# cemlyn007/ale-libtorch-ppo

Hardware: AMD Instinct MI355X
Metric: env steps/sec (whole node), Breakout 84x84x4 (higher is better)
Workload: dtype bf16; 1 GPU; Breakout-shaped synthetic, 128 envs/GPU x T=128, A=4, H=512, 4 epochs x 4 minibatches of 4096 (configs[1], v0.yaml update shape); envs_per_gpu=128, horizon=128, epochs=4, minibatches=4, parallelism=dp1, frames=raw u8 [E,2,210,160] pairs resident in HBM, rollout_planes=fp32, update_graph=False, dp_schedule_forced=False

## Files before the change

### ale-libtorch-ppo_amd/csrc/gemm_launch.hip

```cpp
#include "common.hpp"
#include "gemm.hpp"
#include "gemm_pipe.hpp"
#include <algorithm>
#include <cstdlib>

namespace aleppo {

static int tune(const char *name, int dflt) {
  const char *e = std::getenv(name);
  return e ? std::atoi(e) : dflt;
}
static inline dim3 grid2(long M, int BM, long N, int BN, int Z = 1) {
  return dim3((unsigned)((M + BM - 1) / BM), (unsigned)((N + BN - 1) / BN), (unsigned)Z);
}

template <class T, bool IDX = false>
static void conv1_fwd_t(hipStream_t s, const uint32_t *obs, SampleMap map, const void *W1, const float *b1, void *a1,
                        long ns) {
  if constexpr (!IDX)
    if (map.idx)
      return conv1_fwd_t<T, true>(s, obs, map, W1, b1, a1, ns);
  using AL = ConvGatherLoader<T, uint8_t, 400, 20, 4, 84, 4, 8, IDX>;
  using BL = DenseLoader<T>;
  using EP = EpiBiasAct<T, true>;
  const long M = ns * 400;
  typename AL::P ap{reinterpret_cast<const uint8_t *>(obs), map.TP, map.s1 * 4, map.s0 * 4, map.base * 4, map.n0, map.idx};
  typename BL::P bp{static_cast<const T *>(W1), 256, 0};
  typename EP::P ep{static_cast<T *>(a1), b1, 32, 1.0f / 255.0f};
  hipLaunchKernelGGL((gemm_nt_kernel<T, AL, BL, EP, 128, 32, 4, 1>), grid2(M, 128, 32, 32), dim3(256), 0, s, ap, bp,
                     ep, (int)M, 32, 256);
}
template <class T>
static void conv2_fwd_t(hipStream_t s, const void *a1, const void *W2, const float *b2, void *a2, long ns) {
  using AL = ConvGatherLoader<T, T, 81, 9, 2, 20, 32, 4>;
  using BL = DenseLoader<T>;
  using EP = EpiBiasAct<T, true>;
  const long M = ns * 81;
  typename AL::P ap{static_cast<const T *>(a1), 1, 400 * 32, 0, 0, 0};
  typename BL::P bp{static_cast<const T *>(W2), 512, 0};
  typename EP::P ep{static_cast<T *>(a2), b2, 64, 1.0f};
  hipLaunchKernelGGL((gemm_nt_kernel<T, AL, BL, EP, 128, 64, 2, 2>), grid2(M, 128, 64, 64), dim3(256), 0, s, ap, bp,
                     ep, (int)M, 64, 512);
}
template <class T>
static void conv3_fwd_t(hipStream_t s, const void *a2, const void *W3, const float *b3, void *a3, long ns) {
  using AL = ConvGatherLoader<T, T, 49, 7, 1, 9, 64, 3>;
  using BL = DenseLoader<T>;
  using EP = EpiBiasAct<T, true>;
  const long M = ns * 49;
  typename AL::P ap{static_cast<const T *>(a2), 1, 81 * 64, 0, 0, 0};
  typename BL::P bp{static_cast<const T *>(W3), 576, 0};
  typename EP::P ep{static_cast<T *>(a3), b3, 64, 1.0f};
  hipLaunchKernelGGL((gemm_nt_kernel<T, AL, BL, EP, 128, 64, 2, 2>), grid2(M, 128, 64, 64), dim3(256), 0, s, ap, bp,
                     ep, (int)M, 64, 576);
}

static int pipe_cus() {
  static int n = 0;
  if (!n) {
    int dev = 0;
    hipDeviceProp_t p;
    if (hipGetDevice(&dev) == hipSuccess && hipGetDeviceProperties(&p, dev) == hipSuccess)
      n = p.multiProcessorCount;
    if (n <= 0)
      n = 256;
  }
  return n;
}
template <int MODE, int NST> static void launch_pipe(hipStream_t s, const PipeParams &P) {
  static bool once = false;
  constexpr size_t sm = gemm_pipe_smem<MODE, NST>();
  static_assert(sm <= 160 * 1024, "LDS budget");
  if (!once) {
    (void)hipFuncSetAttribute(reinterpret_cast<const void *>(gemm_pipe_kernel<MODE, NST>),
                              hipFuncAttributeMaxDynamicSharedMemorySize, (int)sm);
    once = true;
  }
  const int cus = pipe_cus() / 8 * 8, rounds = (P.njobs + cus - 1) / cus;
  const int grid = P.njobs >= cus / 4 ? std::min(cus, ((P.njobs + rounds - 1) / rounds + 7) / 8 * 8) : std::min(P.njobs, cus);
  hipLaunchKernelGGL((gemm_pipe_kernel<MODE, NST>), dim3(grid), dim3(PIPE_THREADS), sm, s, P);
}
static bool fc_dma() {
  static const bool v = tune("ALEPPO_FC_DMA", 1) != 0;
  return v;
}
static bool tn_xcd() {
  static const bool v = tune("ALEPPO_TN_XCD", 1) != 0;
  return v;
}
static bool use_pipe() { return tuning().fc_pipe; }
static int fc_fwd_pipe(hipStream_t s, const void *a3, const void *Wfc, const float *bfc, float *h, long ns, int H,
                       int max_parts) {
  const int tm = (int)((ns + 127) / 128), tn = (H + 127) / 128, tiles = tm * tn, cus = pipe_cus();
  int best = 1;
  double best_t = 1e30;
  for (int sp = 1; sp <= max_parts; ++sp) {
    const double t = (double)((tiles * sp + cus - 1) / cus) / sp + 0.02 * sp;
    if (t < best_t - 1e-9) {
      best_t = t;
      best = sp;
    }
  }
  PipeParams P{};
  P.A = static_cast<const bf16 *>(a3);
  P.lda = FC_IN;
  P.B = static_cast<const bf16 *>(Wfc);
  P.ldb = FC_IN;
  P.M = (int)ns;
  P.N = H;
  P.tiles_m = tm;
  P.tiles_n = tn;
  P.nstages = FC_IN / 64;
  P.splits = best;
  P.njobs = tiles * best;
  P.out_f32 = h;
  P.bias = bfc;
  launch_pipe<0, 4>(s, P);
  return best;
}
static void fc_dgrad_pipe(hipStream_t s, const void *dh, const void *WfcT, const void *a3, void *dz3, long ns, int H) {
  PipeParams P{};
  P.A = static_cast<const bf16 *>(dh);
  P.lda = H;
  P.B = static_cast<const bf16 *>(WfcT);
  P.ldb = H;
  P.M = (int)ns;
  P.N = FC_IN;
  P.tiles_m = (int)((ns + 127) / 128);
  P.tiles_n = (FC_IN + 127) / 128;
  P.nstages = H / 64;
  P.splits = 1;
  P.njobs = P.tiles_m * P.tiles_n;
  P.out_bf16 = static_cast<bf16 *>(dz3);
  P.gate = static_cast<const bf16 *>(a3);
  launch_pipe<1, 4>(s, P);
}
template <class T>
static void fc_fwd_t(hipStream_t s, const void *a3, const void *Wfc, const float *bfc, float *h, long ns, int H) {
  using AL = DenseLoader<T>;
  using BL = DenseLoader<T>;
  using EP = EpiBiasAct<float, false>;
  typename AL::P ap{static_cast<const T *>(a3), FC_IN, 0};
  typename BL::P bp{static_cast<const T *>(Wfc), FC_IN, 0};
  typename EP::P ep{h, bfc, H, 1.0f};
  if (ns <= 256)
    hipLaunchKernelGGL((gemm_nt_kernel<T, AL, BL, EP, 32, 32, 2, 2>), grid2(ns, 32, H, 32), dim3(256), 0, s, ap, bp,
                       ep, (int)ns, H, FC_IN);
  else if (fc_dma() && FC_IN % Atom<T>::KT == 0) {
    static const int v = tune("ALEPPO_FC_FWD_TILE", 1);
    const T *a = static_cast<const T *>(a3), *b = static_cast<const T *>(Wfc);
    if (v == 3 && FC_IN % (2 * Atom<T>::KT) == 0)
      hipLaunchKernelGGL((gemm_nt_dma_kernel<T, EP, 64, 64, 2, 2, 16>), grid2(ns, 64, H, 64), dim3(256), 0, s, a, FC_IN,
                         b, FC_IN, ep, (int)ns, H, FC_IN);
    else if (v == 4 && FC_IN % (2 * Atom<T>::KT) == 0)
      hipLaunchKernelGGL((gemm_nt_dma_kernel<T, EP, 128, 64, 2, 2, 16>), grid2(ns, 128, H, 64), dim3(256), 0, s, a,
                         FC_IN, b, FC_IN, ep, (int)ns, H, FC_IN);
    else if (v == 1)
      hipLaunchKernelGGL((gemm_nt_dma_kernel<T, EP, 64, 64, 2, 2>), grid2(ns, 64, H, 64), dim3(256), 0, s, a, FC_IN, b,
                         FC_IN, ep, (int)ns, H, FC_IN);
    else if (v == 2)
      hipLaunchKernelGGL((gemm_nt_dma_kernel<T, EP, 128, 128, 2, 2>), grid2(ns, 128, H, 128), dim3(256), 0, s, a,
                         FC_IN, b, FC_IN, ep, (int)ns, H, FC_IN);
    else
      hipLaunchKernelGGL((gemm_nt_dma_kernel<T, EP, 128, 64, 2, 2>), grid2(ns, 128, H, 64), dim3(256), 0, s, a, FC_IN,
                         b, FC_IN, ep, (int)ns, H, FC_IN);
  } else {
    static const int v = tune("ALEPPO_FC_FWD_TILE", 1);
    if (v == 1)
      hipLaunchKernelGGL((gemm_nt_kernel<T, AL, BL, EP, 64, 64, 2, 2>), grid2(ns, 64, H, 64), dim3(256), 0, s, ap, bp,
                         ep, (int)ns, H, FC_IN);
    else if (v == 2)
      hipLaunchKernelGGL((gemm_nt_kernel<T, AL, BL, EP, 128, 128, 2, 2>), grid2(ns, 128, H, 128), dim3(256), 0, s, ap,
                         bp, ep, (int)ns, H, FC_IN);
    else if (v == 3)
      hipLaunchKernelGGL((gemm_nt_kernel<T, AL, BL, EP, 64, 128, 2, 2>), grid2(ns, 64, H, 128), dim3(256), 0, s, ap,
                         bp, ep, (int)ns, H, FC_IN);
    else
      hipLaunchKernelGGL((gemm_nt_kernel<T, AL, BL, EP, 128, 64, 2, 2>), grid2(ns, 128, H, 64), dim3(256), 0, s, ap,
                         bp, ep, (int)ns, H, FC_IN);
  }
}

template <class T> static void fc_fwd_splitk_t(hipStream_t s, const void *a3, const void *Wfc, float *hpart, long ns, int H) {
  using AL = DenseLoader<T>;
  using BL = DenseLoader<T>;
  using EP = EpiPartial;
  constexpr int KC = FC_IN / FC_SPLITS;
  typename AL::P ap{static_cast<const T *>(a3), FC_IN, KC};
  typename BL::P bp{static_cast<const T *>(Wfc), FC_IN, KC};
  typename EP::P ep{hpart, H, ns * (long)H};
  hipLaunchKernelGGL((gemm_nt_kernel<T, AL, BL, EP, 32, 32, 2, 2>), grid2(ns, 32, H, 32, FC_SPLITS), dim3(256), 0, s,
                     ap, bp, ep, (int)ns, H, KC);
}
__global__ __launch_bounds__(256) void fc_act_kernel(const bf16 *__restrict__ a3, const bf16 *__restrict__ Wfc,
                                                     float *__restrict__ hpart, int M, int N) {
  constexpr int KC = FC_IN / FC_SPLITS, KS = KC / 32, VPR = KC / 8;
  constexpr int ROWV = VPR + 1;
  constexpr int NV = 32 * VPR / 256;
  __shared__ u32x4 sA[32 * ROWV], sB[32 * ROWV];
  const int tid = threadIdx.x, lane = tid & 63, wave = tid >> 6, fr = lane & 15, fg = lane >> 4;
  const int wm = wave >> 1, wn = wave & 1, z = blockIdx.z;
  const int m0 = blockIdx.x * 32, n0 = blockIdx.y * 32;
  u32x4 ra[NV], rb[NV];
#pragma unroll
  for (int i = 0; i < NV; ++i) {
    const int v = tid + 256 * i, r = v / VPR, c = v - r * VPR;
    ra[i] = *reinterpret_cast<const u32x4 *>(a3 + (long)min(m0 + r, M - 1) * FC_IN + z * KC + c * 8);
    rb[i] = *reinterpret_cast<const u32x4 *>(Wfc + (long)min(n0 + r, N - 1) * FC_IN + z * KC + c * 8);
  }
#pragma unroll
  for (int i = 0; i < NV; ++i) {
    const int v = tid + 256 * i, r = v / VPR, c = v - r * VPR;
    sA[r * ROWV + c] = ra[i];
    sB[r * ROWV + c] = rb[i];
  }
  __syncthreads();
  f32x4 acc = {0.f, 0.f, 0.f, 0.f};
#pragma unroll
  for (int ks = 0; ks < KS; ++ks)
    Atom<bf16>::mma(sA[(wm * 16 + fr) * ROWV + ks * 4 + fg], sB[(wn * 16 + fr) * ROWV + ks * 4 + fg], acc);
  float *out = hpart + (long)z * M * N;
  const int nn = n0 + wn * 16 + fr;
#pragma unroll
  for (int r = 0; r < 4; ++r) {
    const int mm = m0 + wm * 16 + fg * 4 + r;
    if (mm < M && nn < N)
      out[(long)mm * N + nn] = acc[r];
  }
}
void fc_fwd_splitk(hipStream_t s, int prec, const void *a3, const void *Wfc, float *hpart, long ns, int H) {
  static const bool latency_form = tune("ALEPPO_FC_ACT_LATENCY", 1) != 0;
  if (prec == ALEPPO_BF16 && latency_form)
    hipLaunchKernelGGL(fc_act_kernel, grid2(ns, 32, H, 32, FC_SPLITS), dim3(256), 0, s, static_cast<const bf16 *>(a3),
                       static_cast<const bf16 *>(Wfc), hpart, (int)ns, H);
  else if (prec == ALEPPO_BF16)
    fc_fwd_splitk_t<bf16>(s, a3, Wfc, hpart, ns, H);
  else
    fc_fwd_splitk_t<float>(s, a3, Wfc, hpart, ns, H);
}

template <class T>
static void fc_dgrad_t(hipStream_t s, const void *dh, const void *WfcT, const void *a3, void *dz3, long ns, int H) {
  using AL = DenseLoader<T>;
  using BL = DenseLoader<T>;
  using EP = EpiReluMask<T, 0>;
  typename AL::P ap{static_cast<const T *>(dh), H, 0};
  typename BL::P bp{static_cast<const T *>(WfcT), H, 0};
  typename EP::P ep{static_cast<T *>(dz3), static_cast<const T *>(a3), FC_IN, 0};
  static const int v = tune("ALEPPO_FC_DGRAD_TILE", 1);
  if (fc_dma() && H % Atom<T>::KT == 0) {
    const T *a = static_cast<const T *>(dh), *b = static_cast<const T *>(WfcT);
    if (v == 3)
      hipLaunchKernelGGL((gemm_nt_dma_kernel<T, EP, 64, 64, 2, 2, 16>), grid2(ns, 64, FC_IN, 64), dim3(256), 0, s, a, H,
                         b, H, ep, (int)ns, FC_IN, H);
    else if (v == 4)
      hipLaunchKernelGGL((gemm_nt_dma_kernel<T, EP, 128, 64, 2, 2, 16>), grid2(ns, 128, FC_IN, 64), dim3(256), 0, s, a,
                         H, b, H, ep, (int)ns, FC_IN, H);
    else if (v == 2)
      hipLaunchKernelGGL((gemm_nt_dma_kernel<T, EP, 128, 128, 2, 2>), grid2(ns, 128, FC_IN, 128), dim3(256), 0, s, a,
                         H, b, H, ep, (int)ns, FC_IN, H);
    else if (v == 0)
      hipLaunchKernelGGL((gemm_nt_dma_kernel<T, EP, 128, 64, 2, 2>), grid2(ns, 128, FC_IN, 64), dim3(256), 0, s, a, H,
                         b, H, ep, (int)ns, FC_IN, H);
    else
      hipLaunchKernelGGL((gemm_nt_dma_kernel<T, EP, 64, 64, 2, 2>), grid2(ns, 64, FC_IN, 64), dim3(256), 0, s, a, H, b,
                         H, ep, (int)ns, FC_IN, H);
    return;
  }
  if (v == 1)
    hipLaunchKernelGGL((gemm_nt_kernel<T, AL, BL, EP, 64, 64, 2, 2>), grid2(ns, 64, FC_IN, 64), dim3(256), 0, s, ap, bp,
                       ep, (int)ns, FC_IN, H);
  else if (v == 2)
    hipLaunchKernelGGL((gemm_nt_kernel<T, AL, BL, EP, 128, 128, 2, 2>), grid2(ns, 128, FC_IN, 128), dim3(256), 0, s,
                       ap, bp, ep, (int)ns, FC_IN, H);
  else
    hipLaunchKernelGGL((gemm_nt_kernel<T, AL, BL, EP, 128, 64, 2, 2>), grid2(ns, 128, FC_IN, 64), dim3(256), 0, s, ap,
                       bp, ep, (int)ns, FC_IN, H);
}
template <class T>
static void conv3_dgrad_t(hipStream_t s, const void *dz3, const void *W3d, const void *a2, void *dz2, long ns) {
  using AL = DgradGatherLoader<T, 9, 9, 7, 7, 64, 3>;
  using BL = DenseLoader<T>;
  using EP = EpiReluMask<T, 0>;
  const long M = ns * 81;
  typename AL::P ap{static_cast<const T *>(dz3)};
  typename BL::P bp{static_cast<const T *>(W3d), 576, 0};
  typename EP::P ep{static_cast<T *>(dz2), static_cast<const T *>(a2), 64, 0};
  hipLaunchKernelGGL((gemm_nt_kernel<T, AL, BL, EP, 128, 64, 2, 2>), grid2(M, 128, 64, 64), dim3(256), 0, s, ap, bp,
                     ep, (int)M, 64, 576);
}
template <class T>
static void conv2_dgrad_t(hipStream_t s, const void *dz2, const void *W2d, const void *a1, void *dz1, long ns) {
  using AL = DgradGatherLoader<T, 10, 10, 9, 9, 64, 2>;
  using BL = DenseLoader<T>;
  using EP = EpiReluMask<T, 1>;
  const long M = ns * 100;
  typename AL::P ap{static_cast<const T *>(dz2)};
  typename BL::P bp{static_cast<const T *>(W2d), 256, 32 * 256};
  typename EP::P ep{static_cast<T *>(dz1), static_cast<const T *>(a1), 32, 0};
  hipLaunchKernelGGL((gemm_nt_kernel<T, AL, BL, EP, 128, 32, 4, 1>), grid2(M, 128, 32, 32, 4), dim3(256), 0, s, ap,
                     bp, ep, (int)M, 32, 256);
}

static inline int pick_slices(long Ktot, int KP, int tiles_mn, int maxS) {
  long S = 512 / tiles_mn;
  const long cap = Ktot / (2L * KP);
  if (S > cap)
    S = cap;
  if (S > maxS)
    S = maxS;
  if (S < 1)
    S = 1;
  return (int)S;
}
static inline int chunk_for(long Ktot, int S, int KP) {
  long c = (Ktot + S - 1) / S;
  c = (c + KP - 1) / KP * KP;
  return (int)c;
}

static int fc_wgrad_split_max() { return tune("ALEPPO_FC_WGRAD_SPLIT", 2); }

template <class T> static int fc_wgrad_t(hipStream_t s, const void *dh, const void *a3, float *sw, float *sb, long ns, int H) {
  using AL = DenseLoader<T>;
  using BL = DenseLoader<T>;
  constexpr int KP = Atom<T>::KT;
  static const int v = tune("ALEPPO_FC_WGRAD_TILE", 0);
  static const int smax = fc_wgrad_split_max();
  const int S = (int)std::max<long>(1, std::min<long>(std::min(smax, MAXS_FC), ns / (4 * KP)));
  const int kc = chunk_for(ns, S, KP);
  typename AL::P ap{static_cast<const T *>(dh), H, 0};
  typename BL::P bp{static_cast<const T *>(a3), FC_IN, 0};
  auto swz = [&](const dim3 &g) { return ((g.x * g.y * S) % 8 == 0 && tn_xcd()) ? (int)(g.x | (g.y << 12)) : 0; };
  auto grid = [&](const dim3 &g, int xsw) { return xsw ? dim3(g.x * g.y * S) : dim3(g.x, g.y, S); };
  if (v == 1) {
    const dim3 g = grid2(H, 64, FC_IN, 64);
    const int xsw = swz(g);
    hipLaunchKernelGGL((gemm_tn_kernel<T, AL, BL, 64, 64, 2, 2, true>), grid(g, xsw), dim3(256), 0, s, ap, bp, sw,
                       sb, H, FC_IN, (int)ns, kc, 1.0f, xsw);
  } else if (v == 2) {
    const dim3 g = grid2(H, 128, FC_IN, 64);
    const int xsw = swz(g);
    hipLaunchKernelGGL((gemm_tn_kernel<T, AL, BL, 128, 64, 2, 2, true>), grid(g, xsw), dim3(256), 0, s, ap, bp,
                       sw, sb, H, FC_IN, (int)ns, kc, 1.0f, xsw);
  } else {
    const dim3 g = grid2(H, 64, FC_IN, 128);
    const int xsw = swz(g);
    hipLaunchKernelGGL((gemm_tn_kernel<T, AL, BL, 64, 128, 2, 2, true>), grid(g, xsw), dim3(256), 0, s, ap, bp,
                       sw, sb, H, FC_IN, (int)ns, kc, 1.0f, xsw);
  }
  return S;
}
template <class T> static int conv3_wgrad_t(hipStream_t s, const void *dz3, const void *a2, float *sw, float *sb, long ns) {
  using AL = DenseLoader<T>;
  using BL = ConvGatherLoader<T, T, 49, 7, 1, 9, 64, 3>;
  constexpr int KP = Atom<T>::KT;
  const long K = ns * 49;
  const dim3 g = grid2(64, 64, 576, 64);
  const int S = pick_slices(K, KP, g.x * g.y, MAXS_C3);
  const int kc = chunk_for(K, S, KP);
  typename AL::P ap{static_cast<const T *>(dz3), 64, 0};
  typename BL::P bp{static_cast<const T *>(a2), 1, 81 * 64, 0, 0, 0};
  hipLaunchKernelGGL((gemm_tn_kernel<T, AL, BL, 64, 64, 2, 2, true>), dim3(g.x, g.y, S), dim3(256), 0, s, ap, bp, sw,
                     sb, 64, 576, (int)K, kc, 1.0f, 0);
  return S;
}
template <class T> static int conv2_wgrad_t(hipStream_t s, const void *dz2, const void *a1, float *sw, float *sb, long ns) {
  using AL = DenseLoader<T>;
  using BL = ConvGatherLoader<T, T, 81, 9, 2, 20, 32, 4>;
  constexpr int KP = Atom<T>::KT;
  const long K = ns * 81;
  const dim3 g = grid2(64, 64, 512, 128);
  const int S = pick_slices(K, KP, g.x * g.y, MAXS_C2);
  const int kc = chunk_for(K, S, KP);
  typename AL::P ap{static_cast<const T *>(dz2), 64, 0};
  typename BL::P bp{static_cast<const T *>(a1), 1, 400 * 32, 0, 0, 0};
  hipLaunchKernelGGL((gemm_tn_kernel<T, AL, BL, 64, 128, 2, 2, true>), dim3(g.x, g.y, S), dim3(256), 0, s, ap, bp, sw,
                     sb, 64, 512, (int)K, kc, 1.0f, 0);
  return S;
}
template <class T, bool IDX = false>
static int conv1_wgrad_t(hipStream_t s, const void *dz1, const uint32_t *obs, SampleMap map, float *sw, float *sb,
                         long ns) {
  if constexpr (!IDX)
    if (map.idx)
      return conv1_wgrad_t<T, true>(s, dz1, obs, map, sw, sb, ns);
  using AL = DenseLoader<T>;
  using BL = ConvGatherLoader<T, uint8_t, 400, 20, 4, 84, 4, 8, IDX>;
  constexpr int KP = Atom<T>::KT;
  const long K = ns * 400;
  const dim3 g = grid2(32, 32, 256, 128);
  const int S = pick_slices(K, KP, g.x * g.y, MAXS_C1);
  const int kc = chunk_for(K, S, KP);
  typename AL::P ap{static_cast<const T *>(dz1), 32, 0};
  typename BL::P bp{reinterpret_cast<const uint8_t *>(obs), map.TP, map.s1 * 4, map.s0 * 4, map.base * 4, map.n0, map.idx};
  hipLaunchKernelGGL((gemm_tn_kernel<T, AL, BL, 32, 128, 1, 4, true>), dim3(g.x, g.y, S), dim3(256), 0, s, ap, bp, sw,
                     sb, 32, 256, (int)K, kc, 1.0f / 255.0f, 0);
  return S;
}

#define DISPATCH(prec, call_f32, call_bf16)                                                                            \
  do {                                                                                                                 \
    if ((prec) == ALEPPO_BF16) {                                                                                       \
      call_bf16;                                                                                                       \
    } else {                                                                                                           \
      call_f32;                                                                                                        \
    }                                                                                                                  \
  } while (0)

void conv1_fwd(hipStream_t s, int prec, const uint32_t *obs, SampleMap map, const void *W1, const float *b1, void *a1,
               long ns) {
  if (prec == ALEPPO_BF16 && use_patch_kernels())
    return patch_conv1_fwd(s, obs, map, W1, b1, a1, ns);
  DISPATCH(prec, conv1_fwd_t<float>(s, obs, map, W1, b1, a1, ns), conv1_fwd_t<bf16>(s, obs, map, W1, b1, a1, ns));
}
void conv2_fwd(hipStream_t s, int prec, const void *a1, const void *W2, const float *b2, void *a2, long ns) {
  if (prec == ALEPPO_BF16 && use_patch_kernels())
    return patch_conv2_fwd(s, a1, W2, b2, a2, ns);
  DISPATCH(prec, conv2_fwd_t<float>(s, a1, W2, b2, a2, ns), conv2_fwd_t<bf16>(s, a1, W2, b2, a2, ns));
}
void conv3_fwd(hipStream_t s, int prec, const void *a2, const void *W3, const float *b3, void *a3, long ns) {
  if (prec == ALEPPO_BF16 && use_patch_kernels())
    return patch_conv3_fwd(s, a2, W3, b3, a3, ns);
  DISPATCH(prec, conv3_fwd_t<float>(s, a2, W3, b3, a3, ns), conv3_fwd_t<bf16>(s, a2, W3, b3, a3, ns));
}
int fc_fwd(hipStream_t s, int prec, const void *a3, const void *Wfc, const float *bfc, float *h, long ns, int H,
           int max_parts) {
  if (prec == ALEPPO_BF16 && ns > 256 && H % 64 == 0 && H >= 64 && use_pipe())
    return fc_fwd_pipe(s, a3, Wfc, bfc, h, ns, H, std::max(1, std::min(max_parts, FC_FWD_MAX_PARTS)));
  DISPATCH(prec, fc_fwd_t<float>(s, a3, Wfc, bfc, h, ns, H), fc_fwd_t<bf16>(s, a3, Wfc, bfc, h, ns, H));
  return 1;
}
void fc_dgrad(hipStream_t s, int prec, const void *dh, const void *WfcT, const void *a3, void *dz3, long ns, int H) {
  if (prec == ALEPPO_BF16 && ns > 256 && H % 64 == 0 && H >= 4 * 64 && use_pipe())
    return fc_dgrad_pipe(s, dh, WfcT, a3, dz3, ns, H);
  DISPATCH(prec, fc_dgrad_t<float>(s, dh, WfcT, a3, dz3, ns, H), fc_dgrad_t<bf16>(s, dh, WfcT, a3, dz3, ns, H));
}
void conv3_dgrad(hipStream_t s, int prec, const void *dz3, const void *W3d, const void *a2, void *dz2, long ns) {
  if (prec == ALEPPO_BF16 && use_patch_kernels())
    return patch_conv3_dgrad(s, dz3, W3d, a2, dz2, ns);
  DISPATCH(prec, conv3_dgrad_t<float>(s, dz3, W3d, a2, dz2, ns), conv3_dgrad_t<bf16>(s, dz3, W3d, a2, dz2, ns));
}
void conv2_dgrad(hipStream_t s, int prec, const void *dz2, const void *W2d, const void *a1, void *dz1, long ns) {
  if (prec == ALEPPO_BF16 && use_patch_kernels())
    return patch_conv2_dgrad(s, dz2, W2d, a1, dz1, ns);
  DISPATCH(prec, conv2_dgrad_t<float>(s, dz2, W2d, a1, dz1, ns), conv2_dgrad_t<bf16>(s, dz2, W2d, a1, dz1, ns));
}
int fc_wgrad_slices(int prec, long ns) {
  static const int smax = fc_wgrad_split_max();
  const int KP = prec == ALEPPO_BF16 ? Atom<bf16>::KT : Atom<float>::KT;
  return (int)std::max<long>(1, std::min<long>(std::min(smax, MAXS_FC), ns / (4 * KP)));
}
int fc_wgrad(hipStream_t s, int prec, const void *dh, const void *a3, float *sw, float *sb, long ns, int H) {
  if (prec == ALEPPO_BF16)
    return fc_wgrad_t<bf16>(s, dh, a3, sw, sb, ns, H);
  return fc_wgrad_t<float>(s, dh, a3, sw, sb, ns, H);
}
int conv3_wgrad(hipStream_t s, int prec, const void *dz3, const void *a2, float *sw, float *sb, long ns) {
  if (prec == ALEPPO_BF16 && use_patch_kernels())
    return patch_conv3_wgrad(s, dz3, a2, sw, sb, ns);
  if (prec == ALEPPO_BF16)
    return conv3_wgrad_t<bf16>(s, dz3, a2, sw, sb, ns);
  return conv3_wgrad_t<float>(s, dz3, a2, sw, sb, ns);
}
int conv2_wgrad(hipStream_t s, int prec, const void *dz2, const void *a1, float *sw, float *sb, long ns) {
  if (prec == ALEPPO_BF16 && use_patch_kernels())
    return patch_conv2_wgrad(s, dz2, a1, sw, sb, ns);
  if (prec == ALEPPO_BF16)
    return conv2_wgrad_t<bf16>(s, dz2, a1, sw, sb, ns);
  return conv2_wgrad_t<float>(s, dz2, a1, sw, sb, ns);
}
int conv1_wgrad(hipStream_t s, int prec, const void *dz1, const uint32_t *obs, SampleMap map, float *sw, float *sb,
                long ns) {
  if (prec == ALEPPO_BF16 && use_patch_kernels())
    return patch_conv1_wgrad(s, dz1, obs, map, sw, sb, ns);
  if (prec == ALEPPO_BF16)
    return conv1_wgrad_t<bf16>(s, dz1, obs, map, sw, sb, ns);
  return conv1_wgrad_t<float>(s, dz1, obs, map, sw, sb, ns);
}

}
```

Measured before the change: 1.508 million env-steps/s.

## Add register-ring pipelined bf16 TN kernel for FC weight gradient

Adds a dedicated bf16 TN GEMM kernel for the FC weight-gradient path. It uses a 128x128 tile and a 4-deep ring of global-load register sets feeding double-buffered LDS, with LDS writes interleaved between MFMA halves to overlap memory with compute. The bias-gradient column sum moves onto extra blocks in the same launch instead of being fused into each GEMM tile, removing redundant reduction work. It becomes the default path when H is divisible by 128, at the cost of heavy register use from the ring and a bespoke kernel to maintain.

```diff
diff --git a/ale-libtorch-ppo_amd/csrc/gemm_launch.hip b/ale-libtorch-ppo_amd/csrc/gemm_launch.hip
--- a/ale-libtorch-ppo_amd/csrc/gemm_launch.hip
+++ b/ale-libtorch-ppo_amd/csrc/gemm_launch.hip
@@ -1,8 +1,10 @@
 #include "common.hpp"
 #include "gemm.hpp"
 #include "gemm_pipe.hpp"
+#include "gemm_tn_ring.hpp"
 #include <algorithm>
 #include <cstdlib>
+#include <type_traits>
 
 namespace aleppo {
 
@@ -333,6 +335,14 @@
   typename BL::P bp{static_cast<const T *>(a3), FC_IN, 0};
   auto swz = [&](const dim3 &g) { return ((g.x * g.y * S) % 8 == 0 && tn_xcd()) ? (int)(g.x | (g.y << 12)) : 0; };
   auto grid = [&](const dim3 &g, int xsw) { return xsw ? dim3(g.x * g.y * S) : dim3(g.x, g.y, S); };
+  if constexpr (std::is_same<T, bf16>::value)
+    if (v == 0 && H % RING_BM == 0) {
+      const dim3 g = grid2(H, RING_BM, FC_IN, RING_BN);
+      const int ngemm = g.x * g.y * S;
+      hipLaunchKernelGGL(gemm_tn_ring_kernel, dim3(ngemm + S * g.x), dim3(256), 0, s, ap.a, bp.a, sw, sb, H, FC_IN,
+                         (int)ns, kc, (int)g.y, S, swz(g) ? 1 : 0);
+      return S;
+    }
   if (v == 1) {
     const dim3 g = grid2(H, 64, FC_IN, 64);
     const int xsw = swz(g);
diff --git a/ale-libtorch-ppo_amd/csrc/gemm_tn_ring.hpp b/ale-libtorch-ppo_amd/csrc/gemm_tn_ring.hpp
--- /dev/null
+++ b/ale-libtorch-ppo_amd/csrc/gemm_tn_ring.hpp
@@ -0,0 +1,188 @@
+#pragma once
+#include "gemm.hpp"
+
+namespace aleppo {
+
+constexpr int RING_BM = 128, RING_BN = 128, RING_KP = 64;
+constexpr int RING_PITCH = RING_BM + KFrag<bf16>::PAD;
+constexpr int RING_TILE = RING_KP * RING_PITCH;
+constexpr int RING_SETS = 4;
+
+__device__ __forceinline__ void ring_bias_sum(const bf16 *__restrict__ A, float *__restrict__ out, int M, int m0, int kbeg,
+                                              int kend, bf16 *sA) {
+  constexpr int KP = RING_KP, SP = RING_PITCH, RV = 4, NS = RING_SETS;
+  const int tid = threadIdx.x, cv = tid & 15, r0 = tid >> 4;
+  const int nk = (kend - kbeg + KP - 1) / KP;
+  const bf16 *const ga = A + m0 + cv * 8;
+  u32x4 ra[NS][RV];
+  float bsum = 0.f;
+  auto gload = [&](int ks, int set) {
+#pragma unroll
+    for (int i = 0; i < RV; ++i)
+      ra[set][i] = *reinterpret_cast<const u32x4 *>(ga + (long)min(kbeg + ks * KP + r0 + 16 * i, kend - 1) * M);
+    __builtin_amdgcn_sched_barrier(0);
+  };
+  auto swrite = [&](int ks, int buf, int set) {
+#pragma unroll
+    for (int i = 0; i < RV; ++i) {
+      const int r = r0 + 16 * i;
+      const bool ok = kbeg + ks * KP + r < kend;
+      *reinterpret_cast<u32x4 *>(&sA[buf * RING_TILE + r * SP + cv * 8]) = ok ? ra[set][i] : zero16();
+    }
+  };
+  auto step = [&](int ks, int j) {
+    gload(ks + NS, j);
+    if (tid < RING_BM) {
+      float s = 0.f;
+#pragma unroll 8
+      for (int p = 0; p < KP; ++p)
+        s += (float)sA[(j & 1) * RING_TILE + p * SP + tid];
+      bsum += s;
+    }
+    swrite(ks + 1, (j + 1) & 1, (j + 1) % NS);
+    __syncthreads();
+  };
+  if (nk > 0) {
+#pragma unroll
+    for (int j = 0; j < NS; ++j)
+      gload(j, j);
+    swrite(0, 0, 0);
+  }
+  __syncthreads();
+  int ks = 0;
+  for (; ks + NS <= nk; ks += NS) {
+#pragma unroll
+    for (int j = 0; j < NS; ++j)
+      step(ks + j, j);
+  }
+#pragma unroll
+  for (int j = 0; j < NS - 1; ++j)
+    if (ks + j < nk)
+      step(ks + j, j);
+  if (tid < RING_BM)
+    out[m0 + tid] = bsum;
+}
+
+__global__ __launch_bounds__(256) void gemm_tn_ring_kernel(const bf16 *__restrict__ A, const bf16 *__restrict__ B,
+                                                            float *__restrict__ slab, float *__restrict__ bias_slab,
+                                                            int M, int N, int Ktot, int kchunk, int gy, int S,
+                                                            int xcd_swizzle) {
+  constexpr int BM = RING_BM, BN = RING_BN, KP = RING_KP, SP = RING_PITCH;
+  constexpr int RV = 4;
+  constexpr int NS = RING_SETS;
+  __shared__ __attribute__((aligned(16))) bf16 lds[4 * RING_TILE];
+  bf16 *const sA = lds, *const sB = lds + 2 * RING_TILE;
+
+  const int tid = threadIdx.x, lane = tid & 63, wave = tid >> 6;
+  const int wm = wave >> 1, wn = wave & 1;
+  const int gx = M / BM, ngemm = gx * gy * S;
+  int w = blockIdx.x;
+  if (w >= ngemm) {
+    const int b = w - ngemm, zb = b / gx, kb = zb * kchunk;
+    ring_bias_sum(A, bias_slab + (long)zb * M, M, (b - zb * gx) * BM, kb, min(Ktot, kb + kchunk), sA);
+    return;
+  }
+  if (xcd_swizzle)
+    w = (w % 8) * (ngemm / 8) + w / 8;
+  const int bx = w % gx, by = (w / gx) % gy, bz = w / (gx * gy);
+  const int m0 = bx * BM, n0 = by * BN, z = bz;
+  const int kbeg = z * kchunk, kend = min(Ktot, kbeg + kchunk);
+  const int nk = (kend - kbeg + KP - 1) / KP;
+
+  const int cv = tid & 15, r0 = tid >> 4;
+  const bf16 *const ga = A + m0 + cv * 8;
+  const bf16 *const gb = B + min(n0 + cv * 8, N - 8);
+
+  f32x4 acc[4][4];
+#pragma unroll
+  for (int i = 0; i < 4; ++i)
+#pragma unroll
+    for (int j = 0; j < 4; ++j)
+      acc[i][j] = f32x4{0.f, 0.f, 0.f, 0.f};
+
+  u32x4 ra[NS][RV], rb[NS][RV];
+  auto gload = [&](int ks, int set) {
+#pragma unroll
+    for (int i = 0; i < RV; ++i)
+      ra[set][i] = *reinterpret_cast<const u32x4 *>(ga + (long)min(kbeg + ks * KP + r0 + 16 * i, kend - 1) * M);
+#pragma unroll
+    for (int i = 0; i < RV; ++i)
+      rb[set][i] = *reinterpret_cast<const u32x4 *>(gb + (long)min(kbeg + ks * KP + r0 + 16 * i, kend - 1) * N);
+    __builtin_amdgcn_sched_barrier(0);
+  };
+  auto swrite_a = [&](int ks, int buf, int set) {
+#pragma unroll
+    for (int i = 0; i < RV; ++i) {
+      const int r = r0 + 16 * i;
+      const bool ok = kbeg + ks * KP + r < kend;
+      *reinterpret_cast<u32x4 *>(&sA[buf * RING_TILE + r * SP + cv * 8]) = ok ? ra[set][i] : zero16();
+    }
+  };
+  auto swrite_b = [&](int ks, int buf, int set) {
+#pragma unroll
+    for (int i = 0; i < RV; ++i) {
+      const int r = r0 + 16 * i;
+      const bool ok = kbeg + ks * KP + r < kend;
+      *reinterpret_cast<u32x4 *>(&sB[buf * RING_TILE + r * SP + cv * 8]) = ok ? rb[set][i] : zero16();
+    }
+  };
+  auto compute = [&](int buf, int kc) {
+    u32x4 fa[4], fb[4];
+#pragma unroll
+    for (int i = 0; i < 4; ++i)
+      fa[i] = KFrag<bf16>::read(sA + buf * RING_TILE, SP, kc * 32, wm * 64 + i * 16, lane);
+#pragma unroll
+    for (int j = 0; j < 4; ++j)
+      fb[j] = KFrag<bf16>::read(sB + buf * RING_TILE, SP, kc * 32, wn * 64 + j * 16, lane);
+#pragma unroll
+    for (int i = 0; i < 4; ++i)
+#pragma unroll
+      for (int j = 0; j < 4; ++j)
+        Atom<bf16>::mma(fa[i], fb[j], acc[i][j]);
+  };
+  auto step = [&](int ks, int j) {
+    gload(ks + NS, j);
+    compute(j & 1, 0);
+    swrite_a(ks + 1, (j + 1) & 1, (j + 1) % NS);
+    compute(j & 1, 1);
+    swrite_b(ks + 1, (j + 1) & 1, (j + 1) % NS);
+    __syncthreads();
+  };
+  static_assert(NS % 2 == 0, "the LDS buffer index is the register set's parity");
+
+  if (nk > 0) {
+#pragma unroll
+    for (int j = 0; j < NS; ++j)
+      gload(j, j);
+    swrite_a(0, 0, 0);
+    swrite_b(0, 0, 0);
+  }
+  __syncthreads();
+  int ks = 0;
+  for (; ks + NS <= nk; ks += NS) {
+#pragma unroll
+    for (int j = 0; j < NS; ++j)
+      step(ks + j, j);
+  }
+#pragma unroll
+  for (int j = 0; j < NS - 1; ++j)
+    if (ks + j < nk)
+      step(ks + j, j);
+
+  const int fr = lane & 15, fg = lane >> 4;
+  float *out = slab + (long)z * M * N;
+#pragma unroll
+  for (int i = 0; i < 4; ++i)
+#pragma unroll
+    for (int r = 0; r < 4; ++r) {
+      const int m = m0 + wm * 64 + i * 16 + fg * 4 + r;
+#pragma unroll
+      for (int j = 0; j < 4; ++j) {
+        const int n = n0 + wn * 64 + j * 16 + fr;
+        if (n < N)
+          out[(long)m * N + n] = acc[i][j][r];
+      }
+    }
+}
+
+}
```

Result: slower. 1.488 million env-steps/s (-1.3%).
